# maurock/small-pathtracer

Measured on AMD Instinct MI355X. Metric: Msamples/sec (w×h×spp/s) on Cornell box; per-channel RMSE vs ref PPM, higher is better.
Workload: dtype f32

## Files before the change

### small-pathtracer_amd/csrc/spt_kernel.hip

```cpp
#include <hip/hip_runtime.h>

#include <utility>

#include "../../include/spt.h"
#include "spt_device.h"
#include "spt_cornell.h"
#include "spt_diag.h"
#include "spt_kparams.h"
#include "spt_variants.h"
#include "spt_launch.h"

#define SPT_STR_(x) #x
#define SPT_XSTR(x) SPT_STR_(x)

namespace spt {

constexpr uint32_t kStIdle = 0;
constexpr uint32_t kStCam = 1;
constexpr uint32_t kStCos = 2;
constexpr uint32_t kStSpec = 3;
constexpr uint32_t kStPath = 4;
constexpr uint32_t kStShadow = 5;
constexpr uint32_t kStTerm = 6;
constexpr uint32_t kStEarly = 7;
constexpr uint32_t kMaxWaveIters = 1u << 26;
#define SPT_CONST __attribute__((address_space(4)))

template <typename T>
__device__ __forceinline__ const SPT_CONST T* cptr(const T* p) {
  asm volatile("" : "+s"(p));
  return (const SPT_CONST T*)p;
}


struct CornellRectPtr {
  int i;
  __device__ constexpr CornellRectPtr operator+(int j) const { return CornellRectPtr{i + j}; }
  __device__ constexpr const CRect* operator->() const { return &kCornellRects[i]; }
};

template <class CF> __device__ __forceinline__ int light_id_of(const SPT_CONST KParams* P) {
  if constexpr (CF::LREF == 1) return kRefLightId; else return P->light_id;
}
template <class TP, class CF> __device__ __forceinline__ int light_slot_of(const SPT_CONST KParams* P) {
  if constexpr (TP::CONSTGEO) return kCornellLightPos; else return light_id_of<CF>(P);
}
template <class CF> __device__ __forceinline__ int rr_depth_of(const SPT_CONST KParams* P) {
  if constexpr (CF::LREF == 1) return kRefRrDepth; else return P->rr_depth;
}
template <class TP>
__device__ __forceinline__ bool unit_dirs_of(const KParams* Pg) {
  if constexpr (TP::DIRS >= 0) {
    (void)Pg;
    return TP::DIRS == 1;
  } else {
    return cptr(Pg)->unit_dirs != 0;
  }
}
template <class TP>
__device__ __forceinline__ auto rects_of(const SPT_CONST SceneGeo* G) {
  if constexpr (TP::CONSTGEO) return CornellRectPtr{0};
  else return G->rect + 0;
}

struct Ray6 { float oa, ia, db, ob, dc, oc; };
template <int AXIS>
__device__ __forceinline__ Ray6 ray6(f3 o, f3 d, float ix, float iy, float iz) {
  if (AXIS == 2) return Ray6{o.z, iz, d.x, o.x, d.y, o.y};
  if (AXIS == 1) return Ray6{o.y, iy, d.x, o.x, d.z, o.z};
  return Ray6{o.x, ix, d.y, o.y, d.z, o.z};
}

constexpr uint32_t kKeyNone = __builtin_bit_cast(uint32_t, 1e20f) | 63u;
constexpr float kNegTiny = -0x1p-149f;
__device__ __forceinline__ float plane_t(float n, float inv) { return fmaf(n, inv, kNegTiny); }
__device__ __forceinline__ uint32_t umin(uint32_t a, uint32_t b) { return a < b ? a : b; }
__device__ __forceinline__ void count_if(uint32_t& c, bool b) {
  const uint64_t m = __builtin_amdgcn_ballot_w64(b);
  asm("v_addc_co_u32_e64 %0, vcc, 0, %0, %1" : "+v"(c) : "s"(m) : "vcc");
}
template <int POS>
__device__ __forceinline__ uint32_t key_c(float t) {
  uint32_t r;
  asm("v_bitop3_b32 %0, %1, %2, 63 bitop3:0x36" : "=v"(r) : "v"(__float_as_uint(t)), "n"(63 - POS));
  return r;
}
__device__ __forceinline__ uint32_t key_v(float t, uint32_t pos) {
  uint32_t r;
  asm("v_bitop3_b32 %0, %1, %2, 63 bitop3:0x36" : "=v"(r) : "v"(__float_as_uint(t)), "v"(63u - pos));
  return r;
}
__device__ __forceinline__ uint32_t key_s(float t, uint32_t pos) {
  uint32_t r;
  asm("v_bitop3_b32 %0, %1, %2, 63 bitop3:0x36" : "=v"(r) : "v"(__float_as_uint(t)), "s"(63u - pos));
  return r;
}

template <int J> struct CornellTestPtr {
  __device__ constexpr const CTest* operator->() const { return &kCornellTests.t[J]; }
};
template <int J, bool PAIR>
__device__ __forceinline__ void plane_keys(CornellTestPtr<J>, float t0, float t1, uint32_t& kp) {
  if constexpr (PAIR) kp = umin(key_c<kCornellTests.t[J].pos0>(t0), key_c<kCornellTests.t[J].pos1>(t1));
  else kp = key_c<kCornellTests.t[J].pos0>(t0);
}
template <int J, bool PAIR>
__device__ __forceinline__ void plane_keys(const GeoTest* g, float t0, float t1, uint32_t& kp) {
  kp = umin(key_v(t0, (uint32_t)g->pos0), key_v(t1, (uint32_t)g->pos1));
}
template <int J, bool PAIR>
__device__ __forceinline__ void plane_keys(const SPT_CONST GeoTest* g, float t0, float t1, uint32_t& kp) {
  kp = umin(key_v(t0, (uint32_t)g->pos0), key_v(t1, (uint32_t)g->pos1));
}
template <int J, bool PAIR, class GP>
__device__ __forceinline__ void rect_cand(GP g, const Ray6& r, uint32_t& tmin) {
  const float t0 = plane_t(g->k0 - r.oa, r.ia);
  float t1 = t0;
  uint32_t kb = __float_as_uint(t0), kp;
  if constexpr (PAIR) {
    t1 = plane_t(g->k1 - r.oa, r.ia);
    kb = umin(kb, __float_as_uint(t1));
  }
  plane_keys<J, PAIR>(g, t0, t1, kp);
  const float tb = __uint_as_float(kb);
  const float a = fmaf(r.db, tb, r.ob - g->ma), b = fmaf(r.dc, tb, r.oc - g->mb);
  const bool inb = (bool)((int)(fabsf(a) <= g->ha) & (int)(fabsf(b) <= g->hb));
  tmin = umin(tmin, inb ? kp : 0xFFFFFFFFu);
}
template <int J>
__device__ __forceinline__ void cornell_test(const Ray6* rays, uint32_t& tmin) {
  constexpr CTest T = kCornellTests.t[J];
  if constexpr (J != kCornellRoom[0] && J != kCornellRoom[1] && J != kCornellRoom[2] && !cornell_in_box(J))
    rect_cand<J, T.pos0 != T.pos1>(CornellTestPtr<J>{}, rays[T.axis], tmin);
}
__device__ __forceinline__ int imin(int a, int b) { return a < b ? a : b; }
__device__ __forceinline__ int imax(int a, int b) { return a > b ? a : b; }
__device__ __forceinline__ void box_keys(int kx0, int kx1, int kz0, int kz1, int ky0, int ky1,
                                         uint32_t& tmin) {
  const int en = imax(imax(imin(kx0, kx1), imin(kz0, kz1)), imin(ky0, ky1));
  const int ex = imin(imin(imax(kx0, kx1), imax(kz0, kz1)), imax(ky0, ky1));
  tmin = umin(tmin, en <= ex ? umin((uint32_t)en, (uint32_t)ex) : 0xFFFFFFFFu);
}
__device__ __forceinline__ void cornell_room(const Ray6* rays, uint32_t& tmin) {
  constexpr CTest Z = kCornellTests.t[kCornellRoom[0]], Y = kCornellTests.t[kCornellRoom[1]];
  constexpr CTest X = kCornellTests.t[kCornellRoom[2]];
  const Ray6 &rz = rays[2], &ry = rays[1], &rx = rays[0];
  box_keys((int)key_c<X.pos0>(plane_t(X.k0 - rx.oa, rx.ia)), (int)key_c<X.pos1>(plane_t(X.k1 - rx.oa, rx.ia)),
           (int)key_c<Z.pos0>(plane_t(Z.k0 - rz.oa, rz.ia)), (int)key_c<Z.pos1>(plane_t(Z.k1 - rz.oa, rz.ia)),
           (int)key_c<Y.pos0>(plane_t(Y.k0 - ry.oa, ry.ia)), (int)key_c<Y.pos1>(plane_t(Y.k1 - ry.oa, ry.ia)),
           tmin);
}
template <int B>
__device__ __forceinline__ void cornell_box(const Ray6* rays, uint32_t& tmin) {
  constexpr CTest Z = kCornellTests.t[kCornellBoxes.t[B][0]], X = kCornellTests.t[kCornellBoxes.t[B][1]];
  constexpr CTest T = kCornellTests.t[kCornellBoxes.t[B][2]], F = kCornellTests.t[kCornellRoom[1]];
  const Ray6 &rz = rays[2], &ry = rays[1], &rx = rays[0];
  box_keys((int)key_c<X.pos0>(plane_t(X.k0 - rx.oa, rx.ia)), (int)key_c<X.pos1>(plane_t(X.k1 - rx.oa, rx.ia)),
           (int)key_c<Z.pos0>(plane_t(Z.k0 - rz.oa, rz.ia)), (int)key_c<Z.pos1>(plane_t(Z.k1 - rz.oa, rz.ia)),
           (int)key_c<F.pos0>(plane_t(F.k0 - ry.oa, ry.ia)), (int)key_c<T.pos0>(plane_t(T.k0 - ry.oa, ry.ia)),
           tmin);
}
template <int... B>
__device__ __forceinline__ void cornell_boxes(std::integer_sequence<int, B...>, const Ray6* rays,
                                              uint32_t& tmin) {
  (cornell_box<B>(rays, tmin), ...);
}
template <class GT>
__device__ __forceinline__ void geo_room(GT rm, const Ray6& rz, const Ray6& ry, const Ray6& rx,
                                         uint32_t& tmin) {
  box_keys((int)key_v(plane_t(rm[2].k0 - rx.oa, rx.ia), (uint32_t)rm[2].pos0),
           (int)key_v(plane_t(rm[2].k1 - rx.oa, rx.ia), (uint32_t)rm[2].pos1),
           (int)key_v(plane_t(rm[0].k0 - rz.oa, rz.ia), (uint32_t)rm[0].pos0),
           (int)key_v(plane_t(rm[0].k1 - rz.oa, rz.ia), (uint32_t)rm[0].pos1),
           (int)key_v(plane_t(rm[1].k0 - ry.oa, ry.ia), (uint32_t)rm[1].pos0),
           (int)key_v(plane_t(rm[1].k1 - ry.oa, ry.ia), (uint32_t)rm[1].pos1), tmin);
}
template <class GT>
__device__ __forceinline__ void geo_box(GT bx, GT fl, const Ray6& rz, const Ray6& ry, const Ray6& rx,
                                        uint32_t& tmin) {
  box_keys((int)key_v(plane_t(bx[1].k0 - rx.oa, rx.ia), (uint32_t)bx[1].pos0),
           (int)key_v(plane_t(bx[1].k1 - rx.oa, rx.ia), (uint32_t)bx[1].pos1),
           (int)key_v(plane_t(bx[0].k0 - rz.oa, rz.ia), (uint32_t)bx[0].pos0),
           (int)key_v(plane_t(bx[0].k1 - rz.oa, rz.ia), (uint32_t)bx[0].pos1),
           (int)key_v(plane_t(fl->k0 - ry.oa, ry.ia), (uint32_t)fl->pos0),
           (int)key_v(plane_t(bx[2].k0 - ry.oa, ry.ia), (uint32_t)bx[2].pos0), tmin);
}
// ... 229 lines not shown
}
__device__ __forceinline__ bool early_nee_proven(f3 x) {
  const int room = early_room_ok(x);
  const int short_box = (int)(x.y >= 25.0f) | (int)(x.x <= 63.0f);
  const int tall_box = (int)(x.y >= 50.0f) | (int)(x.z >= 62.0f);
  return (room & short_box & tall_box) != 0;
}

#ifdef SPT_REGION_STATS
constexpr int kRegions = 10;
#define SPT_REGION(R) (reg_flags |= 1u << (R))
#else
#define SPT_REGION(R) \
  do {                \
  } while (0)
#endif

__device__ __forceinline__ float hit_plane_t(float n, float da, float ia, float t) {
  return fmaf(fmaf(-t, da, n), ia, t);
}
__device__ __forceinline__ float div_nr(float n, float d) { return n * rcp_nr(d); }

__device__ __forceinline__ float nee_weight(bool unit, f3 d, f3 nl, float t, float larea, float nee_c) {
  if (unit) {
    const float pdf = fabsf(div_nr(larea * d.y, t * t));
    const float brdf = fabsf(dot3(d, nl) * 0.318309886183790672f);
    return pdf * brdf;
  }
  const float num = fabsf(d.y) * fabsf(dot3(d, nl));
  const float vv = dot3(d, d);
  return (num * nee_c) * rcp_nr((t * t) * (vv * vv));
}
constexpr float kRefNeeC = (float)(1296.0 / 3.14159265358979323846);


__device__ __forceinline__ uint32_t div_magic(uint32_t n, uint32_t m, uint32_t sh) {
  return (uint32_t)(((uint64_t)n * m) >> sh);
}

__device__ __forceinline__ void pixel_terms(const SPT_CONST KParams* Q, uint32_t lp, PxKey& pk,
                                            float& fx, float& fy) {
  const uint32_t w = (uint32_t)Q->width;
  const uint32_t lr = div_magic(lp, Q->m_w, Q->sh_w);
  const int px = (int)(lp - lr * w);
  const uint32_t T_ = (uint32_t)Q->tile_rows;
  const uint32_t tile = div_magic(lr, Q->m_tile, Q->sh_tile), within = lr - tile * T_;
  const int py = (int)((tile * (uint32_t)Q->shard_count + (uint32_t)Q->shard_index) * T_ + within);
  pk = philox_pixel_key((uint32_t)py * w + (uint32_t)px, Q->seed);
  fx = ((float)px - 0.5f) - 128.0f;
  fy = ((float)(Q->height - py - 1) - 0.5f) - 128.0f;
}

__device__ __forceinline__ void wave_lds_order() {
  __builtin_amdgcn_fence(__ATOMIC_RELEASE, "wavefront");
  __builtin_amdgcn_wave_barrier();
  __builtin_amdgcn_fence(__ATOMIC_ACQUIRE, "wavefront");
}

__device__ __forceinline__ uint32_t lane_rank(uint64_t mask) {
  return __builtin_amdgcn_mbcnt_hi((uint32_t)(mask >> 32),
                                   __builtin_amdgcn_mbcnt_lo((uint32_t)mask, 0u));
}

__device__ __forceinline__ uint32_t unit_pixel(const SPT_CONST KParams* Q, uint32_t u) {
  const uint32_t r = u - div_magic(u, Q->m_npix, Q->sh_npix) * (uint32_t)Q->n_local_pix;
  return (r & ((1u << Q->scr_k) - 1u)) * Q->scr_q + (r >> Q->scr_k);
}

template <class TP, class CF>
#ifndef SPT_NUM_SGPR
#define SPT_NUM_SGPR 80
#endif
__global__ void __launch_bounds__(kBlock) __attribute__((amdgpu_num_sgpr(SPT_NUM_SGPR)))
__attribute__((amdgpu_waves_per_eu((TP::SPH && !TP::MAT && !TP::WIDE) || (!TP::SPH && !TP::MAT && CF::NEE >= 0) ? 8 : 1)))
render_kernel(const KParams* __restrict__ Pg) {
  __shared__ DevPrim s_prims[kMaxPrims];
  __shared__ int s_pos2idx[kMaxPrims];
  __shared__ GeoTest s_test[(TP::CONSTGEO && !TP::UPBOX) || TP::WIDE ? 1 : kMaxPrims];
  struct Node { float o[3], d[3], T[3]; int depth; uint32_t branch; };
  __shared__ Node s_stack[TP::MAT ? kBlock * 2 : 1];
  __shared__ uint32_t s_nsph[TP::SPH ? kBlock / 64 : 1];
  if (TP::SPH && threadIdx.x < kBlock / 64) s_nsph[threadIdx.x] = 0;
  __shared__ uint32_t s_nearly[TP::SPH ? kBlock / 64 : 1];
  if (TP::SPH && threadIdx.x < kBlock / 64) s_nearly[threadIdx.x] = 0;
  constexpr bool kPoolLds = kPoolLdsBuild && !TP::MAT;
  __shared__ PoolEntryA s_pool_a[kPoolLds ? kBlock : 1];
  __shared__ PoolEntryB s_pool_b[kPoolLds ? kBlock : 1];
  {
    const SPT_CONST KParams* P = cptr(Pg);
    const SPT_CONST SceneGeo* G = cptr(P->geo);
    const int nrect = G->n_xy + G->n_xz + G->n_yz;
    for (int i = threadIdx.x; i < P->n_prims; i += kBlock) {
      s_prims[i] = P->prims[TP::CONSTGEO ? G->rect[i].idx : i];
      s_pos2idx[i] = i < nrect ? G->rect[i].idx : G->sph[i - nrect].idx;
      if ((!TP::CONSTGEO || TP::UPBOX) && !TP::WIDE && i < G->n_txy + G->n_txz + G->n_tyz + 3 * G->has_room + 3 * G->n_box) {
        const SPT_CONST GeoTest& q = G->test[i];
        s_test[i] = GeoTest{q.k0, q.k1, q.ma, q.ha, q.mb, q.hb, q.pos0, q.pos1};
      }
    }
  }
  __syncthreads();

  const uint32_t lane = __lane_id();
  uint32_t ls = kStIdle;
  uint32_t branch = 0;
  int sp = 0;
  uint32_t lp = 0, s = 0, s_end = 0;
  PxKey pk = PxKey{0, 0, 0};
  int dp1 = 1, vid = 0;
  float fx = 0.0f, fy = 0.0f;
  float fz = 0.0f;
  unsigned long long acc0 = 0, acc1 = 0, acc2 = 0;
  f3 o = mk(cptr(Pg)->cam[0], cptr(Pg)->cam[1], cptr(Pg)->cam[2]);
  f3 d = mk(0, 0, 1), T = mk(1, 1, 1), L = mk(0, 0, 0), nl = mk(0, 1, 0);
  float w_nee = 0.0f;
  u4 r = u4{0, 0, 0, 0};
  struct CamK { float o0, o1, o2, aux, avy, cux, cvy, lx, ly, lz, fs; };
  CamK ck{};
  if constexpr (CF::CAMAX == 1) {
    const SPT_CONST KParams* C = cptr(Pg);
    ck = CamK{C->cam[0], C->cam[1], C->cam[2], C->cam_au[0], C->cam_av[1], C->cam_cu[0],
              C->cam_cv[1], C->cam_l[0], C->cam_l[1], C->cam_l[2], C->fix_scale};
  }
  struct CamG { float o0, o1, o2, cu0, cu1, cu2, cv0, cv1, cv2, fs; };
  CamG cg{};
  if constexpr (CF::CAMAX == 2) {
    const SPT_CONST KParams* C = cptr(Pg);
    cg = CamG{C->cam[0], C->cam[1], C->cam[2], C->cam_cu[0], C->cam_cu[1], C->cam_cu[2],
              C->cam_cv[0], C->cam_cv[1], C->cam_cv[2], C->fix_scale};
  }
  auto unit_setup = [&](uint32_t u, uint32_t& us, uint32_t& us_end, PxKey& upk, float& ufx, float& ufy,
                        float& ufz) {
    const SPT_CONST KParams* Q = cptr(Pg);
    const uint32_t npix = (uint32_t)Q->n_local_pix;
    const uint32_t j = div_magic(u, Q->m_npix, Q->sh_npix);
    uint32_t up = u - j * npix;
    up = (up & ((1u << Q->scr_k) - 1u)) * Q->scr_q + (up >> Q->scr_k);
    us = Q->s_base + j * (uint32_t)Q->chunk;
    us_end = min(us + (uint32_t)Q->chunk, Q->s_lim);
    pixel_terms(Q, up, upk, ufx, ufy);
    if constexpr (CF::CAMAX == 1) {
      ufx = fmaf(ck.aux, ufx, ck.lx);
      ufy = fmaf(ck.avy, ufy, ck.ly);
    } else if constexpr (CF::CAMAX == 2) {
      const float rx = ufx, ry = ufy;
      ufx = fmaf(Q->cam_au[0], rx, fmaf(Q->cam_av[0], ry, Q->cam_l[0]));
      ufy = fmaf(Q->cam_au[1], rx, fmaf(Q->cam_av[1], ry, Q->cam_l[1]));
      ufz = fmaf(Q->cam_au[2], rx, fmaf(Q->cam_av[2], ry, Q->cam_l[2]));
    }
  };
  const uint32_t pool_lds = kPoolLds ? (uint32_t)__builtin_amdgcn_readfirstlane((int)(threadIdx.x & ~63u)) : 0u;
  uint32_t pool_next = 0, pool_end = 0, grab_at = 0;
  bool exhausted = false, capped = false;
  uint32_t n_path = 0, n_cos = 0;
  using KT = KernelTraits<TP, CF>;
  constexpr bool kNeeByIdentity = KT::kNeeByIdentity, kEarlyNee = KT::kEarlyNee,
                 kEarlySph = KT::kEarlySph, kEarlyGeo = KT::kEarlyGeo, kEarly = KT::kEarly;
  uint32_t l_early = 0;
  uint32_t l_miss = 0, l_nee = 0, l_hit = 0;
  uint32_t l_shadow = 0;
#ifdef SPT_REGION_STATS
  uint32_t reg_exec[kRegions] = {}, reg_lanes[kRegions] = {};
  uint32_t reg_flags = 0;
#endif

#ifdef SPT_WAVE_TIMES
  const unsigned long long wave_t0 = __builtin_amdgcn_s_memrealtime();
  uint32_t wave_iters = 0;
#endif
  for (uint32_t iter = 0;; ++iter) {
#ifdef SPT_WAVE_TIMES
    wave_iters = iter;
#endif
    const SPT_CONST KParams* P = cptr(Pg);
    SPT_REGION(0);
    if (__builtin_expect(iter >= kMaxWaveIters, 0)) {
      capped = true;
      exhausted = true;
      ls = kStIdle;
    }
    uint64_t need = __ballot(ls == kStIdle);
    if (need != 0) {
    bool needs_unit = ls == kStIdle;
    while (need != 0 && !exhausted) {
      SPT_REGION(2);
      const SPT_CONST KParams* Q = cptr(Pg);
      if (pool_next >= pool_end) {
        uint32_t want = kGrab;
        if (Q->sh_guided < 32u) {
          const uint32_t left = Q->n_units - min(grab_at, (uint32_t)Q->n_units);
          want = min(kGrab, max(max((uint32_t)__popcll(need), kGrabMin), left >> Q->sh_guided));
        }
        if (blockIdx.x >= Q->young_block) {
          uint32_t q = 0;
          if (lane == 0) q = __hip_atomic_load(Q->queue, __ATOMIC_RELAXED, __HIP_MEMORY_SCOPE_AGENT);
          q = __builtin_amdgcn_readfirstlane(q);
          if (q >= Q->young_cut) { exhausted = true; break; }
        }
        uint32_t b = 0;
        if (lane == 0) b = atomicAdd(Q->queue, want);
        b = __builtin_amdgcn_readfirstlane(b);
        grab_at = b + want;
        if (b >= Q->n_units) { exhausted = true; break; }
        pool_next = b;
        pool_end = min(b + want, Q->n_units);
        if constexpr (kPoolLds) {
          wave_lds_order();
          const uint32_t u = b + lane;
          if (u < pool_end) {
            uint32_t us, us_end;
            PxKey upk;
            float ufx, ufy, ufz = 0.0f;
            unit_setup(u, us, us_end, upk, ufx, ufy, ufz);
            s_pool_a[pool_lds + (u & 63u)] = PoolEntryA{us, upk.qhi, upk.qlo, upk.lo};
            if constexpr (CF::CAMAX != 2) ufz = __uint_as_float(u | 0x80000000u);
            s_pool_b[pool_lds + (u & 63u)] = PoolEntryB{ufx, ufy, ufz, us_end};
          }
          wave_lds_order();
        }
      }
      const uint32_t rank = lane_rank(need);
      const uint32_t avail = pool_end - pool_next;
      if (needs_unit && rank < avail) {
        const uint32_t u = pool_next + rank;
        if constexpr (kPoolLds) {
          const PoolEntryA ea = s_pool_a[pool_lds + (u & 63u)];
          const PoolEntryB eb = s_pool_b[pool_lds + (u & 63u)];
          s = ea.s;
          pk = PxKey{ea.qhi, ea.qlo, ea.lo};
          fx = eb.fx;
          fy = eb.fy;
          s_end = eb.s_end;
          if constexpr (CF::CAMAX == 2) {
            fz = eb.fz;
            lp = u | 0x80000000u;
          } else {
            lp = __float_as_uint(eb.fz);
          }
        } else {
          unit_setup(u, s, s_end, pk, fx, fy, fz);
          lp = u | 0x80000000u;
        }
        ls = kStCam;
        needs_unit = false;
      }
      pool_next += min((uint32_t)__popcll(need), avail);
      need = __ballot(needs_unit);
    }
    if (exhausted) {
      uint64_t idle = __ballot(ls == kStIdle);
      if (idle != 0) {
        const uint32_t cur = s + (ls == kStCam ? 0u : 1u);
        const uint32_t smin = cptr(Pg)->steal_min;
        uint64_t dm = __ballot(ls != kStIdle && s_end > cur + (ls == kStCam ? 1u : 0u) &&
                               s_end >= cur + smin);
        while (idle != 0 && dm != 0) {
          const int il = __builtin_ctzll(idle), dl = __builtin_ctzll(dm);
          idle &= idle - 1;
          dm &= dm - 1;
          const uint32_t dcur = (uint32_t)__builtin_amdgcn_readlane((int)cur, dl);
          const uint32_t dend = (uint32_t)__builtin_amdgcn_readlane((int)s_end, dl);
          const uint32_t mid = dcur + (dend - dcur) / 2u;
          uint32_t d_lp = (uint32_t)__builtin_amdgcn_readlane((int)lp, dl);
          if (d_lp >> 31)
            d_lp = unit_pixel(cptr(Pg), d_lp & 0x7FFFFFFFu);
          const uint32_t d_qhi = (uint32_t)__builtin_amdgcn_readlane((int)pk.qhi, dl);
          const uint32_t d_qlo = (uint32_t)__builtin_amdgcn_readlane((int)pk.qlo, dl);
          const uint32_t d_lo = (uint32_t)__builtin_amdgcn_readlane((int)pk.lo, dl);
          const float d_fx = __int_as_float(__builtin_amdgcn_readlane(__float_as_int(fx), dl));
          const float d_fy = __int_as_float(__builtin_amdgcn_readlane(__float_as_int(fy), dl));
          float d_fz = 0.0f;
          if constexpr (CF::CAMAX == 2) d_fz = __int_as_float(__builtin_amdgcn_readlane(__float_as_int(fz), dl));
          const bool tk = lane == (uint32_t)il;
          s_end = tk ? dend : (lane == (uint32_t)dl ? mid : s_end);
          s = tk ? mid : s;
          lp = tk ? d_lp : lp;
          pk.qhi = tk ? d_qhi : pk.qhi;
          pk.qlo = tk ? d_qlo : pk.qlo;
          pk.lo = tk ? d_lo : pk.lo;
          fx = tk ? d_fx : fx;
          fy = tk ? d_fy : fy;
          if constexpr (CF::CAMAX == 2) fz = tk ? d_fz : fz;
          ls = tk ? kStCam : ls;
        }
      }
    }
    if (__ballot(ls != kStIdle) == 0) break;
    }
    n_cos += (uint32_t)__popcll(__ballot(ls == kStCos));

    if (ls - kStCam < 3u) {
      const bool cam = ls == kStCam;
      if (ls != kStSpec) SPT_REGION(cam ? 3 : 8);
      const bool unit = unit_dirs_of<TP>(Pg);
      f3 v = cosine_vec<!TP::SPH>(nl, r.z, r.w, TP::MAT && cptr(Pg)->scatter_uniform != 0, unit);
      const uint32_t ctr2 = (uint32_t)dp1 | (TP::MAT ? branch << 24 : 0u);
      r = philox_px(pk, s, ctr2);
      {
        const SPT_CONST KParams* C = cptr(Pg);
        f3 vc;
        const float Fu = jitter_f(r.x, r.y), Fv = jitter_f(r.z, r.w);
        if constexpr (CF::CAMAX == 1) {
          vc = mk(fmaf(Fu, ck.cux, fx), fmaf(Fv, ck.cvy, fy), ck.lz);
        } else if constexpr (CF::CAMAX == 2) {
          vc = mk(fmaf(Fv, cg.cv0, fmaf(Fu, cg.cu0, fx)), fmaf(Fv, cg.cv1, fmaf(Fu, cg.cu1, fy)),
                  fmaf(Fv, cg.cv2, fmaf(Fu, cg.cu2, fz)));
        } else {
          float vv[3];
#pragma unroll
          for (int c = 0; c < 3; ++c) {
            const float Pc = fmaf(C->cam_au[c], fx, fmaf(C->cam_av[c], fy, C->cam_l[c]));
            vv[c] = fmaf(Fv, C->cam_cv[c], fmaf(Fu, C->cam_cu[c], Pc));
          }
          vc = mk(vv[0], vv[1], vv[2]);
        }
        v = mk(cam ? vc.x : v.x, cam ? vc.y : v.y, cam ? vc.z : v.z);
      }
      const f3 dn = normalize_dir(v, unit);
      if constexpr (TP::MAT) {
        const bool kd = ls == kStSpec;
        d = mk(kd ? d.x : dn.x, kd ? d.y : dn.y, kd ? d.z : dn.z);
      } else {
        d = dn;
      }
      ls = kStPath;
    }

    if constexpr (TP::MAT) n_path += (uint32_t)__popcll(__ballot(ls == kStPath));
    if constexpr (TP::SPH) l_shadow += (uint32_t)__popcll(__ballot(ls == kStShadow));
    if (ls >= kStPath) {
      SPT_REGION(4);
#ifdef SPT_PROBE_SALU
      { uint32_t z_ = iter; asm volatile(".rept " SPT_XSTR(SPT_PROBE_SALU) "\n s_add_u32 %0, %0, 1\n .endr" : "+s"(z_)); }
#endif
#ifdef SPT_PROBE_VALU
      { float z_ = o.x; asm volatile(".rept " SPT_XSTR(SPT_PROBE_VALU) "\n v_add_f32 %0, 1.0, %0\n .endr" : "+v"(z_)); }
#endif
      const SPT_CONST SceneGeo* G = TP::CONSTGEO && !TP::UPLIGHT ? nullptr : cptr(P->geo);
      int id = (!kEarlyNee && ls == kStShadow) ? vid : 0;
      float t = 0.0f, ia_hit = 0.0f;
      int hpos;
      f3 inv;
      bool hit = intersect_scene<TP, kEarly>(G, rects_of<TP>(G), tests_of<TP>(G, s_test), G->sph, s_pos2idx,
                                             o, d, id, ia_hit, hpos, l_miss, inv);
      if constexpr (TP::CONSTGEO)
        ia_hit = hpos < kCornellNXY ? inv.z : (hpos < kCornellNXY + kCornellNXZ ? inv.y : inv.x);

      const bool traced_shadow = ls == kStShadow;
      if (!kEarly && ls == kStShadow) {
        SPT_REGION(6);
        const SPT_CONST KParams* D = cptr(Pg);
        const bool lh = id == light_slot_of<TP, CF>(D);
        if (lh) SPT_REGION(7);
        count_if(l_hit, lh);
        if constexpr (!TP::SPH) ++l_shadow;
        const float larea = CF::LREF == 1 ? kRefLarea : D->larea;
        const float nee_c = CF::LREF == 1 ? kRefNeeC : D->nee_c;
        t = hit_t<TP>(s_prims[id], hpos, o, d, ia_hit, G);
        const float w = lh ? nee_weight(unit_dirs_of<TP>(Pg), d, nl, t, larea, nee_c) : 1.0f;
        T = mk(T.x * w, T.y * w, T.z * w);
        if (CF::BLACK != 1 && lh && !(hit && s_prims[id].pmax == 0.0f))
          r = philox_px(pk, s, (uint32_t)dp1 | (TP::MAT ? branch << 24 : 0u));
        ls = lh ? kStPath : kStCos;
      }

      if (ls == kStPath) {
        SPT_REGION(5);
        const DevPrim& H = s_prims[id];
        const int kind = H.kind;
        f3 x;
        f3 gn = mk(0, 0, 0);
        bool ax_xy = false, ax_xz = false;
        if constexpr (!TP::SPH) {
          bool kxy, kxz;
          if constexpr (TP::CONSTGEO) {
            kxy = hpos < kCornellNXY;
            kxz = !kxy && hpos < kCornellNXY + kCornellNXZ;
          } else {
            kxy = kind == SPT_RECT_XY;
            kxz = kind == SPT_RECT_XZ;
          }
          ax_xy = kxy;
          ax_xz = kxz;
          const bool kyz = !kxy && !kxz;
          const float oa = kxy ? o.z : (kxz ? o.y : o.x);
          const float da = kxy ? d.z : (kxz ? d.y : d.x);
          const float n_ = H.w1 - oa;
          float ia = ia_hit;
          if constexpr (TP::CONSTGEO) ia = kxy ? inv.z : (kxz ? inv.y : inv.x);
          const float tr = hit_plane_t(n_, da, ia, plane_t(n_, ia));
          x = mk(keep(o.x + d.x * tr), keep(o.y + d.y * tr), keep(o.z + d.z * tr));
          if constexpr (CF::LEAK != 1) x = hit ? x : mk(0, 0, 0);
          if constexpr (!kEarly) l_miss += hit ? 0u : 1u;
          const float sg = da < 0.0f ? 1.0f : -1.0f;
          nl = mk(kyz ? sg : 0.0f, kxz ? sg : 0.0f, kxy ? sg : 0.0f);
          if (TP::MAT) gn = mk(kyz ? 1.0f : 0.0f, kxz ? 1.0f : 0.0f, kxy ? 1.0f : 0.0f);
        } else {
        if (!hit) {
          x = mk(0, 0, 0);
          if constexpr (!kEarly) ++l_miss;
        } else {
          float tr = hit_t<TP>(H, hpos, o, d, ia_hit, G);
          if (kind == SPT_RECT_XY) tr = hit_plane_t(H.w1 - o.z, d.z, ia_hit, tr);
          else if (kind == SPT_RECT_XZ) tr = hit_plane_t(H.w1 - o.y, d.y, ia_hit, tr);
          else if (kind == SPT_RECT_YZ) tr = hit_plane_t(H.w1 - o.x, d.x, ia_hit, tr);
          x = mk(o.x + d.x * tr, o.y + d.y * tr, o.z + d.z * tr);
        }
        if (kind == SPT_RECT_XY) {
          nl = d.z < 0.0f ? mk(0, 0, 1) : mk(0, 0, -1);
          if (TP::MAT) gn = mk(0, 0, 1);
        } else if (kind == SPT_RECT_XZ) {
          nl = d.y < 0.0f ? mk(0, 1, 0) : mk(0, -1, 0);
          if (TP::MAT) gn = mk(0, 1, 0);
        } else if (kind == SPT_RECT_YZ) {
          nl = d.x < 0.0f ? mk(1, 0, 0) : mk(-1, 0, 0);
          if (TP::MAT) gn = mk(1, 0, 0);
        } else {
          const f3 n = mk((x.x - H.w1) * H.w5, (x.y - H.w2) * H.w5, (x.z - H.w3) * H.w5);
          nl = dot3(n, d) < 0.0f ? n : mk(-n.x, -n.y, -n.z);
          if (TP::MAT) gn = n;
          atomicAdd(&s_nsph[threadIdx.x / 64], 1u);
        }
        }
        f3 f = mk(H.cx, H.cy, H.cz);
        const f3 e = mk(H.ex, H.ey, H.ez);
        const int rr_t = H.rr_t;
        const int depth = dp1++;
        u4 rl = r;
        if (CF::NOS1 != 1 && depth == 1) {
          const SPT_CONST KParams* C = cptr(Pg);
          if (C->rr_depth < 1 || (C->nee_prob > 0.0f && C->nee_prob < 1.0f))
            rl = philox_px(pk, s, 1u | 0x80000000u);
        }
        const int max_depth = CF::MAXD0 == 1 ? 0 : P->max_depth;
        const bool capd = (max_depth > 0) & (depth >= max_depth);
        const bool rr = (depth > rr_depth_of<CF>(P)) | (rr_t < 0);
        const bool alive = (int)u16i(rl.x, rl.y) < rr_t;
        const bool leak = CF::LEAK == 1 || (CF::LEAK < 0 && P->leak_end != 0);
        const bool term = capd | (rr & !alive) | (!hit & leak);
        const float ip = keep(H.ip);
        const float fsc = rr ? ip : 1.0f;
        f = mk(f.x * fsc, f.y * fsc, f.z * fsc);
        L = mk(fmaf(T.x, e.x, L.x), fmaf(T.y, e.y, L.y), fmaf(T.z, e.z, L.z));
        T = mk(T.x * f.x, T.y * f.y, T.z * f.z);
        o = x;
        if constexpr (!kEarlyNee) vid = id;
        uint32_t nxt = kStCos;
        if (TP::MAT && !term && H.refl != SPT_DIFF) {
          const f3 Tf = T;
          const float k2 = 2.0f * dot3(gn, d);
          const f3 refl = mk(d.x - gn.x * k2, d.y - gn.y * k2, d.z - gn.z * k2);
          bool use_refl = true;
          if (H.refl == SPT_REFR) {
            const bool into = dot3(gn, nl) > 0.0f;
            const float nnt = into ? 1.0f / 1.5f : 1.5f / 1.0f;
            const float ddn = dot3(d, nl);
            const float cos2t = 1.0f - nnt * nnt * (1.0f - ddn * ddn);
            if (!(cos2t < 0.0f)) {
              const float kk = (into ? 1.0f : -1.0f) * (ddn * nnt + sqrtf(cos2t));
              const f3 tdir = normalize3(mk(d.x * nnt - gn.x * kk, d.y * nnt - gn.y * kk,
                                            d.z * nnt - gn.z * kk));
              const float a = 1.5f - 1.0f, b = 1.5f + 1.0f, R0 = a * a / (b * b);
              const float c = 1.0f - (into ? -ddn : dot3(tdir, gn));
              const float Re = R0 + (1.0f - R0) * c * c * c * c * c, Tr = 1.0f - Re;
              const float Pp = 0.25f + 0.5f * Re, RP = Re / Pp, TP_ = Tr / (1.0f - Pp);
              if (depth > 2) {
                if (u16(rl.z, rl.w) < Pp) {
                  T = mk(Tf.x * RP, Tf.y * RP, Tf.z * RP);
                } else {
                  T = mk(Tf.x * TP_, Tf.y * TP_, Tf.z * TP_);
                  d = tdir;
                  use_refl = false;
                }
              } else {
                Node& N = s_stack[threadIdx.x * 2 + sp];
                N.o[0] = x.x; N.o[1] = x.y; N.o[2] = x.z;
                N.d[0] = tdir.x; N.d[1] = tdir.y; N.d[2] = tdir.z;
                N.T[0] = Tf.x * Tr; N.T[1] = Tf.y * Tr; N.T[2] = Tf.z * Tr;
                N.depth = depth;
                N.branch = branch | (1u << (depth - 1));
                ++sp;
                T = mk(Tf.x * Re, Tf.y * Re, Tf.z * Re);
              }
            }
          }
          if (use_refl) d = refl;
          nxt = kStSpec;
        } else {
          const SPT_CONST KParams* D = cptr(Pg);
          bool nee;
          if constexpr (CF::NEE == 1) {
            nee = true;
          } else if constexpr (CF::NEE == 0) {
            nee = false;
          } else {
            const float q = D->nee_prob;
            if (q >= 1.0f) nee = true;
            else if (q <= 0.0f) nee = false;
            else nee = u16(rl.z, rl.w) < q;
          }
          if (nee) {
            float xl, zl;
            const int lmode = CF::LMODE >= 0 ? CF::LMODE : D->light_mode;
            if (lmode == SPT_LIGHT_GLIBC_WRAP) {
              const uint32_t ldxi = CF::LREF == 1 ? kRefLdxi : D->ldxi;
              const uint32_t ldzi = CF::LREF == 1 ? kRefLdzi : D->ldzi;
              const float lx0 = CF::LREF == 1 ? kRefLx0 : D->lx0, lz0 = CF::LREF == 1 ? kRefLz0 : D->lz0;
              if constexpr (CF::LREF == 1) {
                static_assert(kRefLdxi == 36u && kRefLdzi == 36u, "LREF light lattice");
                xl = fmaf(__uint_as_float(0x4B000000u | (r.x >> 9)), 0x1p-22f, lx0 - 3.0f);
                zl = fmaf(__uint_as_float(0x4B000000u | (r.y >> 9)), 0x1p-22f, lz0 - 3.0f);
              } else {
                xl = D->lx_lattice ? fmaf((float)(r.x >> D->lx_shift), D->lx_scale, D->lx0m1)
                                   : fmaf((float)(int32_t)(((r.x >> 8) << 7) * ldxi), 0x1p-31f, lx0);
                zl = D->lz_lattice ? fmaf((float)(r.y >> D->lz_shift), D->lz_scale, D->lz0m1)
                                   : fmaf((float)(int32_t)(((r.y >> 8) << 7) * ldzi), 0x1p-31f, lz0);
              }
            } else {
              xl = fmaf(u01(r.x), D->ldx, D->lx0);
              zl = fmaf(u01(r.y), D->ldz, D->lz0);
            }
            const float ly = CF::LREF == 1 ? kRefLy : D->ly;
            const f3 vl = mk(xl - x.x, ly - x.y, zl - x.z);
            const f3 dl = unit_dirs_of<TP>(Pg) ? normalize3(vl) : vl;
            if constexpr (!kNeeByIdentity) l_nee += term ? 0u : 1u;
            const SPT_CONST SceneGeo* G2 = TP::CONSTGEO ? nullptr : cptr(D->geo);
            bool la, early = false;
            if constexpr (kEarlyNee) {
              const Ray6 rl6{x.y, rcp_nr(dl.y), dl.x, x.x, dl.z, x.z};
              RectHit h;
              if constexpr (TP::UPLIGHT) h = rect_eval_test(cptr(D->geo)->test[0], rl6);
              else h = rect_eval(CornellRectPtr{kCornellLightPos}, rl6);
              la = h.inb & key_valid(h.tt, kCornellLightPos);
              if constexpr (TP::UPLIGHT) early = la & early_geo_proven<1>(x, D);
              else if constexpr (TP::UPBOX) early = la & early_geo_proven<0>(x, D);
              else early = la & early_nee_proven(x);
              const float adot = fabsf(ax_xy ? dl.z : (ax_xz ? dl.y : dl.x));
              const float num = fabsf(dl.y) * adot;
              const float vv = dot3(dl, dl);
              w_nee = (num * kRefNeeC) * rcp_nr((h.tt * h.tt) * (vv * vv));
            } else if constexpr (kEarlySph || kEarlyGeo) {
              const RectHit h = rect_eval(G2->rect + D->light_pos,
                                          Ray6{x.y, rcp_nr(dl.y), dl.x, x.x, dl.z, x.z});
              la = h.inb & key_valid(h.tt, (uint32_t)D->light_pos);
              if constexpr (kEarlySph) early = la & early_room_proven(x, D->early_y0);
              else early = la & early_geo_proven<2>(x, D);
              t = early ? h.tt : t;
            } else {
              la = light_accepts<TP>(D, G2, rects_of<TP>(G2), x, dl);
            }
            const bool cand = (id == light_slot_of<TP, CF>(D)) | la;
            d = dl;
            nxt = early ? kStEarly : (cand ? kStShadow : kStCos);
          }
        }
        ls = term ? kStTerm : nxt;
      }
      if constexpr (kEarly) {
        if (traced_shadow || ls == kStEarly) {
          SPT_REGION(6);
          const bool ea = ls == kStEarly;
          const bool th = id == light_slot_of<TP, CF>(cptr(Pg));
          const bool lh = ea | th;
          if (lh) SPT_REGION(7);
          count_if(l_hit, th);
          if constexpr (TP::SPH) {
            if (ea) atomicAdd(&s_nearly[threadIdx.x / 64], 1u);
          } else {
            l_early += ea ? 1u : 0u;
            ++l_shadow;
          }
          float wl;
          if constexpr (kEarlyNee) {
            wl = w_nee;
          } else {
            const float kl = s_prims[light_slot_of<TP, CF>(cptr(Pg))].w1;
            const float tl = ea ? t : plane_t(kl - o.y, ia_hit);
            wl = keep(nee_weight(unit_dirs_of<TP>(Pg), d, nl, tl, kRefLarea, kRefNeeC));
          }
          const float wh = lh ? wl : 0.0f;
          const f3 Tw = mk(T.x * wh, T.y * wh, T.z * wh);
          const DevPrim& H = s_prims[light_slot_of<TP, CF>(cptr(Pg))];
          L = mk(fmaf(Tw.x, H.ex, L.x), fmaf(Tw.y, H.ey, L.y), fmaf(Tw.z, H.ez, L.z));
          ls = lh ? kStTerm : kStCos;
        }
      }
      if (ls == kStTerm) {
        if (TP::MAT && sp > 0) {
          --sp;
          const Node& N = s_stack[threadIdx.x * 2 + sp];
          o = mk(N.o[0], N.o[1], N.o[2]);
          d = mk(N.d[0], N.d[1], N.d[2]);
          T = mk(N.T[0], N.T[1], N.T[2]);
          dp1 = N.depth + 1;
          branch = N.branch;
          ls = kStSpec;
        } else {
          SPT_REGION(9);
          const float scale = CF::CAMAX == 1 ? ck.fs : (CF::CAMAX == 2 ? cg.fs : cptr(Pg)->fix_scale);
          acc0 += fix31(L.x, scale);
          acc1 += fix31(L.y, scale);
          acc2 += fix31(L.z, scale);
          ++s;
          L = mk(0, 0, 0);
          T = mk(1, 1, 1);
          dp1 = 1;
          {
            const SPT_CONST KParams* C = cptr(Pg);
            o = CF::CAMAX == 1   ? mk(ck.o0, ck.o1, ck.o2)
                : CF::CAMAX == 2 ? mk(cg.o0, cg.o1, cg.o2)
                                 : mk(C->cam[0], C->cam[1], C->cam[2]);
          }
          if (TP::MAT) branch = 0;
          ls = kStCam;
          if (s >= s_end) {
            SPT_REGION(1);
            if (lp >> 31) {
              unsigned long long* a = cptr(Pg)->slots + 3ull * (lp & 0x7FFFFFFFu);
              a[0] = acc0;
              a[1] = acc1;
              a[2] = acc2;
            } else {
              unsigned long long* a = cptr(Pg)->accum + 3ull * lp;
              if (acc0) atomicAdd(a + 0, acc0);
              if (acc1) atomicAdd(a + 1, acc1);
              if (acc2) atomicAdd(a + 2, acc2);
            }
            acc0 = acc1 = acc2 = 0;
            ls = kStIdle;
          }
        }
      }
    }
#ifdef SPT_REGION_STATS
#pragma unroll
    for (int k = 0; k < kRegions; ++k) {
      const uint64_t m = __ballot((reg_flags >> k) & 1u);
      reg_exec[k] += m != 0;
      reg_lanes[k] += (uint32_t)__popcll(m);
    }
    reg_flags = 0;
#endif
  }
  {
    unsigned long long* st = cptr(Pg)->stats;
#ifdef SPT_WAVE_TIMES
    if (lane == 0) {
      const unsigned long long t1 = __builtin_amdgcn_s_memrealtime(), dt = t1 - wave_t0;
      atomicAdd(st + 12, dt);
      atomicAdd(st + 13, dt * dt);
      atomicMin(st + 14, wave_t0);
      atomicMax(st + 15, t1);
      atomicAdd(st + 16, (unsigned long long)wave_iters);
      atomicMax(st + 17, (unsigned long long)wave_iters);
      atomicAdd(st + 18, wave_t0 >> 4);
      atomicAdd(st + 19, t1 >> 4);
      atomicAdd(st + 20, (unsigned long long)__smid());
      const uint32_t wid = blockIdx.x * (kBlock / 64) + threadIdx.x / 64;
      if (wid < 32768) {
        st[32 + 3 * wid] = wave_t0;
        st[33 + 3 * wid] = t1;
        st[34 + 3 * wid] = ((unsigned long long)__smid() << 32) | wave_iters;
      }
    }
#endif
#ifdef SPT_REGION_STATS
    if (lane == 0) {
      for (int k = 0; k < kRegions; ++k) {
        atomicAdd(st + kStatRegion + 2 * k, (unsigned long long)reg_exec[k]);
        atomicAdd(st + kStatRegion + 1 + 2 * k, (unsigned long long)reg_lanes[k]);
      }
    }
#endif
    if (lane == 0) {
      if (capped) atomicAdd(st + 0, 1ull);
      const unsigned long long np = TP::MAT ? n_path : n_cos;
      atomicAdd(st + 1, np);
      atomicAdd(st + 3, np);
      atomicAdd(st + 6, (unsigned long long)n_cos);
    }
    if (!TP::MAT && blockIdx.x == 0 && threadIdx.x == 0) {
      const SPT_CONST KParams* C = cptr(Pg);
      const unsigned long long samples = (unsigned long long)C->n_local_pix * (unsigned long long)C->s_count;
      atomicAdd(st + 1, samples);
      atomicAdd(st + 3, samples);
    }
    {
      if constexpr (!kNeeByIdentity) {
        atomicAdd(st + 2, (unsigned long long)l_nee);
        atomicAdd(st + 4, (unsigned long long)l_nee);
      }
      if constexpr (kEarlyNee || kEarlyGeo) l_hit += l_early;
      atomicAdd(st + 3, (unsigned long long)l_hit);
      atomicAdd(st + 5, (unsigned long long)l_hit);
      atomicAdd(st + 7, (unsigned long long)l_miss);
      if constexpr (TP::SPH) {
        if (lane == 0) atomicAdd(st + kStatShadowTraced, (unsigned long long)l_shadow);
      } else {
        atomicAdd(st + kStatShadowTraced, (unsigned long long)l_shadow);
      }
      if constexpr (TP::SPH)
        if (lane == 0) atomicAdd(st + kStatSphereVertices, (unsigned long long)s_nsph[threadIdx.x / 64]);
      if constexpr (kEarlyNee || kEarlyGeo) atomicAdd(st + kStatShadowProven, (unsigned long long)l_early);
      if constexpr (kEarlySph) {
        if (lane == 0) {
          const unsigned long long ne = s_nearly[threadIdx.x / 64];
          atomicAdd(st + kStatShadowProven, ne);
          atomicAdd(st + kStatShadowTraced, ne);
          atomicAdd(st + 3, ne);
          atomicAdd(st + 5, ne);
        }
      }
    }
  }
}
__global__ void __launch_bounds__(kBlock)
finalize_slots_kernel(const unsigned long long* __restrict__ accum,
                      const unsigned long long* __restrict__ slots, float* __restrict__ rgb,
                      uint32_t npix, uint32_t n_chunks, uint32_t scr_k, uint32_t scr_q,
                      const unsigned long long* __restrict__ stats) {
  const uint32_t t = blockIdx.x * kBlock + threadIdx.x;
  if (t >= npix) return;
  const uint32_t p = (t & ((1u << scr_k) - 1u)) * scr_q + (t >> scr_k);
  if (stats[0] != 0) {
    rgb[3ull * p] = rgb[3ull * p + 1] = rgb[3ull * p + 2] = __builtin_nanf("");
    return;
  }
  unsigned long long v0 = accum[3ull * p], v1 = accum[3ull * p + 1], v2 = accum[3ull * p + 2];
  for (uint32_t j = 0; j < n_chunks; ++j) {
    const unsigned long long* q = slots + 3ull * ((size_t)j * npix + t);
    v0 += q[0];
    v1 += q[1];
    v2 += q[2];
  }
  const float f0 = (float)v0 * 0x1p-31f, f1 = (float)v1 * 0x1p-31f, f2 = (float)v2 * 0x1p-31f;
  rgb[3ull * p] = f0 > 1.0f ? 1.0f : f0;
  rgb[3ull * p + 1] = f1 > 1.0f ? 1.0f : f1;
  rgb[3ull * p + 2] = f2 > 1.0f ? 1.0f : f2;
}

using RenderFn = void (*)(const KParams*);
#define SPT_X_FN(id, name, TP, CF, level, young) render_kernel<TP, CF>,
static const RenderFn kRenderKernels[KV_COUNT] = {SPT_KERNEL_VARIANTS(SPT_X_FN)};
#undef SPT_X_FN

int render_kernel_occupancy(int kv) {
  int bpc = 0;
  if (hipOccupancyMaxActiveBlocksPerMultiprocessor(&bpc, kRenderKernels[kv], kBlock, 0) != hipSuccess)
    return 0;
  return bpc;
}

void launch_render_kernel(int kv, int grid, const KParams* kp_dev, void* stream) {
  hipLaunchKernelGGL(kRenderKernels[kv], dim3(grid), dim3(kBlock), 0, (hipStream_t)stream, kp_dev);
}

void launch_finalize_slots(const unsigned long long* accum, const unsigned long long* slots,
                           float* rgb, uint32_t npix, uint32_t n_chunks, uint32_t scr_k,
                           uint32_t scr_q, const unsigned long long* stats, void* stream) {
  hipLaunchKernelGGL(finalize_slots_kernel, dim3((npix + kBlock - 1) / kBlock), dim3(kBlock), 0,
                     (hipStream_t)stream, accum, slots, rgb, npix, n_chunks, scr_k, scr_q, stats);
}

}
```

Before: 42860.

## Restructure wave loop control, refill path, and stats counting in path kernel

Replaces the inner refill while-loop with a single-pass refill per iteration. The iteration cap becomes a countdown that also serves as the loop exit, so the per-iteration cap check disappears. Scalar-pinned constant pointer reloads (cptr_at) are tied to the loop counter to steer compiler scheduling and register use, the shadow flag is made wave-uniform via ballot, and the depth increment is moved. Stats counting is altered so non-material variants count generated camera/cos/spec states. The changes risk subtle behaviour shifts: refill takes extra iterations when more lanes need units, and the stats semantics change.

```diff
diff --git a/small-pathtracer_amd/csrc/spt_kernel.hip b/small-pathtracer_amd/csrc/spt_kernel.hip
--- a/small-pathtracer_amd/csrc/spt_kernel.hip
+++ b/small-pathtracer_amd/csrc/spt_kernel.hip
@@ -31,7 +31,11 @@
   asm volatile("" : "+s"(p));
   return (const SPT_CONST T*)p;
 }
-
+template <int SITE, typename T>
+__device__ __forceinline__ const SPT_CONST T* cptr_at(const T* p, uint32_t it) {
+  asm("" : "+s"(p) : "s"(it), "n"(SITE));
+  return (const SPT_CONST T*)p;
+}
 
 struct CornellRectPtr {
   int i;
@@ -567,7 +571,7 @@
   const uint32_t pool_lds = kPoolLds ? (uint32_t)__builtin_amdgcn_readfirstlane((int)(threadIdx.x & ~63u)) : 0u;
   uint32_t pool_next = 0, pool_end = 0, grab_at = 0;
   bool exhausted = false, capped = false;
-  uint32_t n_path = 0, n_cos = 0;
+  uint32_t n_path = 0, n_cos = 0, n_gen = 0;
   using KT = KernelTraits<TP, CF>;
   constexpr bool kNeeByIdentity = KT::kNeeByIdentity, kEarlyNee = KT::kEarlyNee,
                  kEarlySph = KT::kEarlySph, kEarlyGeo = KT::kEarlyGeo, kEarly = KT::kEarly;
@@ -583,84 +587,88 @@
   const unsigned long long wave_t0 = __builtin_amdgcn_s_memrealtime();
   uint32_t wave_iters = 0;
 #endif
-  for (uint32_t iter = 0;; ++iter) {
+  uint32_t left = kMaxWaveIters;
+  constexpr bool kExitAtRefill = TP::SPH && !TP::MAT && CF::NEE < 0;
+  bool live = true;
+  for (;;) {
+    [[maybe_unused]] const uint32_t iter = kMaxWaveIters - left;
 #ifdef SPT_WAVE_TIMES
     wave_iters = iter;
 #endif
-    const SPT_CONST KParams* P = cptr(Pg);
+    const SPT_CONST KParams* P = cptr_at<0>(Pg, left);
     SPT_REGION(0);
-    if (__builtin_expect(iter >= kMaxWaveIters, 0)) {
-      capped = true;
-      exhausted = true;
-      ls = kStIdle;
-    }
-    uint64_t need = __ballot(ls == kStIdle);
+    const uint64_t need = __ballot(ls == kStIdle);
     if (need != 0) {
-    bool needs_unit = ls == kStIdle;
-    while (need != 0 && !exhausted) {
+    if (!exhausted) {
       SPT_REGION(2);
       const SPT_CONST KParams* Q = cptr(Pg);
       if (pool_next >= pool_end) {
         uint32_t want = kGrab;
         if (Q->sh_guided < 32u) {
-          const uint32_t left = Q->n_units - min(grab_at, (uint32_t)Q->n_units);
-          want = min(kGrab, max(max((uint32_t)__popcll(need), kGrabMin), left >> Q->sh_guided));
-        }
+          const uint32_t rest = Q->n_units - min(grab_at, (uint32_t)Q->n_units);
+          want = min(kGrab, max(max((uint32_t)__popcll(need), kGrabMin), rest >> Q->sh_guided));
+        }
+        bool open = true;
         if (blockIdx.x >= Q->young_block) {
           uint32_t q = 0;
           if (lane == 0) q = __hip_atomic_load(Q->queue, __ATOMIC_RELAXED, __HIP_MEMORY_SCOPE_AGENT);
           q = __builtin_amdgcn_readfirstlane(q);
-          if (q >= Q->young_cut) { exhausted = true; break; }
-        }
-        uint32_t b = 0;
-        if (lane == 0) b = atomicAdd(Q->queue, want);
-        b = __builtin_amdgcn_readfirstlane(b);
-        grab_at = b + want;
-        if (b >= Q->n_units) { exhausted = true; break; }
-        pool_next = b;
-        pool_end = min(b + want, Q->n_units);
-        if constexpr (kPoolLds) {
-          wave_lds_order();
-          const uint32_t u = b + lane;
-          if (u < pool_end) {
-            uint32_t us, us_end;
-            PxKey upk;
-            float ufx, ufy, ufz = 0.0f;
-            unit_setup(u, us, us_end, upk, ufx, ufy, ufz);
-            s_pool_a[pool_lds + (u & 63u)] = PoolEntryA{us, upk.qhi, upk.qlo, upk.lo};
-            if constexpr (CF::CAMAX != 2) ufz = __uint_as_float(u | 0x80000000u);
-            s_pool_b[pool_lds + (u & 63u)] = PoolEntryB{ufx, ufy, ufz, us_end};
+          open = q < Q->young_cut;
+        }
+        if (open) {
+          uint32_t b = 0;
+          if (lane == 0) b = atomicAdd(Q->queue, want);
+          b = __builtin_amdgcn_readfirstlane(b);
+          grab_at = b + want;
+          open = b < Q->n_units;
+          if (open) {
+            pool_next = b;
+            pool_end = min(b + want, Q->n_units);
+            if constexpr (kPoolLds) {
+              wave_lds_order();
+              const uint32_t u = b + lane;
+              if (u < pool_end) {
+                uint32_t us, us_end;
+                PxKey upk;
+                float ufx, ufy, ufz = 0.0f;
+                unit_setup(u, us, us_end, upk, ufx, ufy, ufz);
+                s_pool_a[pool_lds + (u & 63u)] = PoolEntryA{us, upk.qhi, upk.qlo, upk.lo};
+                if constexpr (CF::CAMAX != 2) ufz = __uint_as_float(u | 0x80000000u);
+                s_pool_b[pool_lds + (u & 63u)] = PoolEntryB{ufx, ufy, ufz, us_end};
+              }
+              wave_lds_order();
+            }
           }
-          wave_lds_order();
-        }
-      }
-      const uint32_t rank = lane_rank(need);
-      const uint32_t avail = pool_end - pool_next;
-      if (needs_unit && rank < avail) {
-        const uint32_t u = pool_next + rank;
-        if constexpr (kPoolLds) {
-          const PoolEntryA ea = s_pool_a[pool_lds + (u & 63u)];
-          const PoolEntryB eb = s_pool_b[pool_lds + (u & 63u)];
-          s = ea.s;
-          pk = PxKey{ea.qhi, ea.qlo, ea.lo};
-          fx = eb.fx;
-          fy = eb.fy;
-          s_end = eb.s_end;
-          if constexpr (CF::CAMAX == 2) {
-            fz = eb.fz;
+        }
+        exhausted = !open;
+      }
+      if (!exhausted) {
+        const uint32_t rank = lane_rank(need);
+        const uint32_t avail = pool_end - pool_next;
+        if (ls == kStIdle && rank < avail) {
+          const uint32_t u = pool_next + rank;
+          if constexpr (kPoolLds) {
+            const PoolEntryA ea = s_pool_a[pool_lds + (u & 63u)];
+            const PoolEntryB eb = s_pool_b[pool_lds + (u & 63u)];
+            s = ea.s;
+            pk = PxKey{ea.qhi, ea.qlo, ea.lo};
+            fx = eb.fx;
+            fy = eb.fy;
+            s_end = eb.s_end;
+            if constexpr (CF::CAMAX == 2) {
+              fz = eb.fz;
+              lp = u | 0x80000000u;
+            } else {
+              lp = __float_as_uint(eb.fz);
+            }
+          } else {
+            unit_setup(u, s, s_end, pk, fx, fy, fz);
             lp = u | 0x80000000u;
-          } else {
-            lp = __float_as_uint(eb.fz);
           }
-        } else {
-          unit_setup(u, s, s_end, pk, fx, fy, fz);
-          lp = u | 0x80000000u;
-        }
-        ls = kStCam;
-        needs_unit = false;
-      }
-      pool_next += min((uint32_t)__popcll(need), avail);
-      need = __ballot(needs_unit);
+          ls = kStCam;
+        }
+        pool_next += min((uint32_t)__popcll(need), avail);
+      }
     }
     if (exhausted) {
       uint64_t idle = __ballot(ls == kStIdle);
@@ -700,9 +708,16 @@
         }
       }
     }
-    if (__ballot(ls != kStIdle) == 0) break;
-    }
-    n_cos += (uint32_t)__popcll(__ballot(ls == kStCos));
+    if (__ballot(ls != kStIdle) == 0) {
+      live = false;
+      left = 1;
+    }
+    }
+    if constexpr (kExitAtRefill) {
+      if (!live) break;
+    }
+    if constexpr (TP::MAT) n_cos += (uint32_t)__popcll(__ballot(ls == kStCos));
+    else n_gen += (uint32_t)__popcll(__ballot(ls - kStCam < 3u));
 
     if (ls - kStCam < 3u) {
       const bool cam = ls == kStCam;
@@ -712,7 +727,7 @@
       const uint32_t ctr2 = (uint32_t)dp1 | (TP::MAT ? branch << 24 : 0u);
       r = philox_px(pk, s, ctr2);
       {
-        const SPT_CONST KParams* C = cptr(Pg);
+        const SPT_CONST KParams* C = cptr_at<1>(Pg, left);
         f3 vc;
         const float Fu = jitter_f(r.x, r.y), Fv = jitter_f(r.z, r.w);
         if constexpr (CF::CAMAX == 1) {
@@ -740,6 +755,7 @@
       }
       ls = kStPath;
     }
+    ls = keep(ls);
 
     if constexpr (TP::MAT) n_path += (uint32_t)__popcll(__ballot(ls == kStPath));
     if constexpr (TP::SPH) l_shadow += (uint32_t)__popcll(__ballot(ls == kStShadow));
@@ -761,10 +777,15 @@
       if constexpr (TP::CONSTGEO)
         ia_hit = hpos < kCornellNXY ? inv.z : (hpos < kCornellNXY + kCornellNXZ ? inv.y : inv.x);
 
-      const bool traced_shadow = ls == kStShadow;
+      bool traced_shadow = ls == kStShadow;
+      if constexpr (kEarly) {
+        uint64_t tsm = __ballot(ls == kStShadow);
+        asm volatile("" : "+s"(tsm));
+        traced_shadow = __builtin_amdgcn_inverse_ballot_w64(tsm);
+      }
       if (!kEarly && ls == kStShadow) {
         SPT_REGION(6);
-        const SPT_CONST KParams* D = cptr(Pg);
+        const SPT_CONST KParams* D = cptr_at<2>(Pg, left);
         const bool lh = id == light_slot_of<TP, CF>(D);
         if (lh) SPT_REGION(7);
         count_if(l_hit, lh);
@@ -840,10 +861,10 @@
         f3 f = mk(H.cx, H.cy, H.cz);
         const f3 e = mk(H.ex, H.ey, H.ez);
         const int rr_t = H.rr_t;
-        const int depth = dp1++;
+        const int depth = dp1;
         u4 rl = r;
         if (CF::NOS1 != 1 && depth == 1) {
-          const SPT_CONST KParams* C = cptr(Pg);
+          const SPT_CONST KParams* C = cptr_at<3>(Pg, left);
           if (C->rr_depth < 1 || (C->nee_prob > 0.0f && C->nee_prob < 1.0f))
             rl = philox_px(pk, s, 1u | 0x80000000u);
         }
@@ -902,7 +923,7 @@
           if (use_refl) d = refl;
           nxt = kStSpec;
         } else {
-          const SPT_CONST KParams* D = cptr(Pg);
+          const SPT_CONST KParams* D = cptr_at<4>(Pg, left);
           bool nee;
           if constexpr (CF::NEE == 1) {
             nee = true;
@@ -970,12 +991,13 @@
           }
         }
         ls = term ? kStTerm : nxt;
+        dp1 = depth + 1;
       }
       if constexpr (kEarly) {
         if (traced_shadow || ls == kStEarly) {
           SPT_REGION(6);
           const bool ea = ls == kStEarly;
-          const bool th = id == light_slot_of<TP, CF>(cptr(Pg));
+          const bool th = id == light_slot_of<TP, CF>(cptr_at<5>(Pg, left));
           const bool lh = ea | th;
           if (lh) SPT_REGION(7);
           count_if(l_hit, th);
@@ -989,13 +1011,13 @@
           if constexpr (kEarlyNee) {
             wl = w_nee;
           } else {
-            const float kl = s_prims[light_slot_of<TP, CF>(cptr(Pg))].w1;
+            const float kl = s_prims[light_slot_of<TP, CF>(cptr_at<6>(Pg, left))].w1;
             const float tl = ea ? t : plane_t(kl - o.y, ia_hit);
             wl = keep(nee_weight(unit_dirs_of<TP>(Pg), d, nl, tl, kRefLarea, kRefNeeC));
           }
           const float wh = lh ? wl : 0.0f;
           const f3 Tw = mk(T.x * wh, T.y * wh, T.z * wh);
-          const DevPrim& H = s_prims[light_slot_of<TP, CF>(cptr(Pg))];
+          const DevPrim& H = s_prims[light_slot_of<TP, CF>(cptr_at<7>(Pg, left))];
           L = mk(fmaf(Tw.x, H.ex, L.x), fmaf(Tw.y, H.ey, L.y), fmaf(Tw.z, H.ez, L.z));
           ls = lh ? kStTerm : kStCos;
         }
@@ -1021,7 +1043,7 @@
           T = mk(1, 1, 1);
           dp1 = 1;
           {
-            const SPT_CONST KParams* C = cptr(Pg);
+            const SPT_CONST KParams* C = cptr_at<8>(Pg, left);
             o = CF::CAMAX == 1   ? mk(ck.o0, ck.o1, ck.o2)
                 : CF::CAMAX == 2 ? mk(cg.o0, cg.o1, cg.o2)
                                  : mk(C->cam[0], C->cam[1], C->cam[2]);
@@ -1056,7 +1078,9 @@
     }
     reg_flags = 0;
 #endif
-  }
+    if (--left == 0) break;
+  }
+  capped = live;
   {
     unsigned long long* st = cptr(Pg)->stats;
 #ifdef SPT_WAVE_TIMES
@@ -1089,16 +1113,15 @@
 #endif
     if (lane == 0) {
       if (capped) atomicAdd(st + 0, 1ull);
-      const unsigned long long np = TP::MAT ? n_path : n_cos;
+      const unsigned long long np = TP::MAT ? n_path : n_gen;
       atomicAdd(st + 1, np);
       atomicAdd(st + 3, np);
-      atomicAdd(st + 6, (unsigned long long)n_cos);
+      atomicAdd(st + 6, (unsigned long long)(TP::MAT ? n_cos : n_gen));
     }
     if (!TP::MAT && blockIdx.x == 0 && threadIdx.x == 0) {
       const SPT_CONST KParams* C = cptr(Pg);
       const unsigned long long samples = (unsigned long long)C->n_local_pix * (unsigned long long)C->s_count;
-      atomicAdd(st + 1, samples);
-      atomicAdd(st + 3, samples);
+      atomicAdd(st + 6, 0ull - samples);
     }
     {
       if constexpr (!kNeeByIdentity) {
```

After: 43410 (median of 6 runs). +1.3%, better.
